# OpenHardware-Initiative/Drone-OA-IREE-ViT-Accelerator

Measured on AMD Instinct MI355X. Metric: frames/s on ITAViTLSTM int8, 60x90 depth input, higher is better.
Workload: dtype int8+f32; 1 GPU; ITAViTLSTM int8 end-to-end forward (BASELINE config 4): 1024 synthetic 60x90 depth frames per GPU per step, LSTM state carried, velocity all-gather; frames_per_gpu=1024, global_batch=1024, parallelism=dp1, image_dtype=u8, weights=seed-0 synthetic QAT (tests/golden), gather_every=1, gather=none (one GPU), schedule=one stream

## Files before the change

### drone-oa-iree-vit-accelerator_amd/csrc/ita_f16x3_kernels.h

```cpp
#pragma once
#include <type_traits>
#include "ita_device.h"

typedef _Float16 f16x8 __attribute__((ext_vector_type(8)));
typedef _Float16 f16x4 __attribute__((ext_vector_type(4)));
typedef float f32x16 __attribute__((ext_vector_type(16)));

__device__ __forceinline__ void split_f16(float x, _Float16& hi, _Float16& lo) {
  hi = (_Float16)x;
  lo = (_Float16)(x - (float)hi);
}

struct ItaGemmSplitArgs {
  const _Float16 *a_hi, *a_lo; int lda;
  const _Float16 *w_hi, *w_lo; int ldw;
  float* out;
  int M, N, K;
  int nsplit;
  int dbg;
  const _Float16 *wf_hi, *wf_lo;
};

template <int ROWS, int NT>
__device__ __forceinline__ void stage_plane(const _Float16* __restrict__ g, int ld, int row0, int max_row, int k0,
// ... 255 lines not shown
  }
  f32x4 xlast0 = {0.0f, 0.0f, 0.0f, 0.0f};
  float xlast1 = 0.0f;
  if (h == 0) {
    const f32x4 q = *(const f32x4*)(a.quat + (size_t)bc * 4);
    xlast0 = (f32x4){a.desvel[bc] / 10.0f, q.x, q.y, q.z};
    xlast1 = q.w;
  }
  const f32x4 ci = *(const f32x4*)(a.c_in + sb * 128 + u0);
  const f32x4 nh = *(const f32x4*)(a.nx_h_in + sb * 128 + u0);
  f32x4 bz[4];
#pragma unroll
  for (int gt = 0; gt < 4; ++gt) bz[gt] = *(const f32x4*)(a.bias + gt * 128 + u0);
  __builtin_amdgcn_sched_barrier(0);
#pragma unroll
  for (int i = 0; i < 4; ++i) {
    f32x4 ps = pz[0][i];
#pragma unroll
    for (int z = 1; z < NS; ++z) ps += pz[z][i];
    *(f32x4*)&pt[8 * i + (lane >> 3)][4 * (lane & 7)] = ps;
  }
#pragma unroll
  for (int i = 0; i < 16; ++i) *(f32x4*)&hs[2 * i + h][4 * r] = hv[i];
  __syncthreads();
#pragma unroll
  for (int s = 0; s < 9; ++s) {
    f32x4 x0 = xlast0, x1 = {xlast1, 0.0f, 0.0f, 0.0f};
    if (s < 8) {
      x0 = *(const f32x4*)&hs[r][16 * s + 8 * h];
      x1 = *(const f32x4*)&hs[r][16 * s + 8 * h + 4];
    }
    f16x8 xh, xl;
#pragma unroll
    for (int j = 0; j < 8; ++j) {
      const float x = j < 4 ? x0[j & 3] : x1[j & 3];
      const _Float16 hi = (_Float16)x;
      xh[j] = hi;
      xl[j] = (_Float16)(x - (float)hi);
    }
    acc = __builtin_amdgcn_mfma_f32_32x32x16_f16(wl[s], xh, acc, 0, 0, 0);
    acc = __builtin_amdgcn_mfma_f32_32x32x16_f16(wh[s], xl, acc, 0, 0, 0);
    acc = __builtin_amdgcn_mfma_f32_32x32x16_f16(wh[s], xh, acc, 0, 0, 0);
  }
  if (b >= a.B) return;
  f32x4 hn, cn;
#pragma unroll
  for (int q = 0; q < 4; ++q) {
    float g[4];
#pragma unroll
    for (int gt = 0; gt < 4; ++gt)
      g[gt] = (pt[r][gt * 8 + 4 * h + q] * a.inv_fold_scale + acc[4 * gt + q] * a.inv_wscale) + bz[gt][q];
    const float ig = lstm_sigmoid_fast(g[0]), fg = lstm_sigmoid_fast(g[1]), cg = lstm_tanh_fast(g[2]), og = lstm_sigmoid_fast(g[3]);
    const float c = fmaf(fg, ci[q], ig * cg);
    cn[q] = c;
    hn[q] = og * lstm_tanh_fast(c);
  }
  *(f32x4*)(a.c_out + sb * 128 + u0) = cn;
  *(f32x4*)(a.h_out + sb * 128 + u0) = hn;
  f16x4 h_hi, h_lo, n_hi, n_lo;
#pragma unroll
  for (int q = 0; q < 4; ++q) {
    _Float16 x, y;
    split_f16(hn[q], x, y); h_hi[q] = x; h_lo[q] = y;
    split_f16(nh[q], x, y); n_hi[q] = x; n_lo[q] = y;
  }
  const size_t o0 = ita_lstm_plane_index(b, u0), o1 = ita_lstm_plane_index(b, 128 + u0);
  *(f16x4*)(a.nx_hi + o0) = h_hi;
  *(f16x4*)(a.nx_lo + o0) = h_lo;
  *(f16x4*)(a.nx_hi + o1) = n_hi;
  *(f16x4*)(a.nx_lo + o1) = n_lo;
}

struct ItaLstmLayerArgs {
  const _Float16 *a_hi, *a_lo; int lda;
  const _Float16 *w_hi, *w_lo; int ldw;
  float inv_wscale;
  const float* bsum;
  const float* c_in;
  float *h_out, *c_out;
  _Float16 *nx_hi, *nx_lo;
  const float* nx_h_in;
  int B, K;
  const int* slots;
};
template <int NK>
__global__ __launch_bounds__(256) void ita_lstm_layer_kernel(const ItaLstmLayerArgs a) {
  __shared__ float part[4][16][64];
  const int tid = threadIdx.x, lane = tid & 63, wave = tid >> 6;
  const int ut = blockIdx.x, f0 = blockIdx.y * 32;
  static_assert(NK == 4, "fragment-order operands: four k-ranges of four k-steps (K = 256)");
  const size_t ao = ((size_t)((blockIdx.y * 4 + wave) * 4) * 64 + lane) * 8;
  const size_t wo = ((size_t)((ut * 4 + wave) * 4) * 64 + lane) * 8;
  f16x8 fah[NK], fal[NK], fwh[NK], fwl[NK];
#pragma unroll
  for (int s = 0; s < NK; ++s) {
    fwh[s] = *(const f16x8*)(a.w_hi + wo + 512 * s);
    fah[s] = *(const f16x8*)(a.a_hi + ao + 512 * s);
    fwl[s] = *(const f16x8*)(a.w_lo + wo + 512 * s);
    fal[s] = *(const f16x8*)(a.a_lo + ao + 512 * s);
  }
  const int ef = tid >> 3, eu = tid & 7;
  const int b = f0 + ef, u = ut * 8 + eu;
  const size_t sb = a.slots ? (size_t)a.slots[min(b, a.B - 1)] : (size_t)min(b, a.B - 1);
  const float c_prev = a.c_in[sb * 128 + u];
  const float nx_prev = a.nx_hi ? a.nx_h_in[sb * 128 + u] : 0.0f;
  const float b_i = a.bsum[u], b_f = a.bsum[128 + u], b_g = a.bsum[256 + u], b_o = a.bsum[384 + u];
  __builtin_amdgcn_sched_barrier(0);
  f32x16 acc;
#pragma unroll
  for (int e = 0; e < 16; ++e) acc[e] = 0.0f;
#pragma unroll
  for (int s = 0; s < NK; ++s) {
    acc = __builtin_amdgcn_mfma_f32_32x32x16_f16(fwl[s], fah[s], acc, 0, 0, 0);
    acc = __builtin_amdgcn_mfma_f32_32x32x16_f16(fwh[s], fal[s], acc, 0, 0, 0);
    acc = __builtin_amdgcn_mfma_f32_32x32x16_f16(fwh[s], fah[s], acc, 0, 0, 0);
  }
#pragma unroll
  for (int e = 0; e < 16; ++e) part[wave][e][lane] = acc[e];
  __syncthreads();
  if (b >= a.B) return;
  float gsum[4];
  const int pl = ef + 32 * (eu >> 2);
#pragma unroll
  for (int gte = 0; gte < 4; ++gte) {
    const int e = 4 * gte + (eu & 3);
    gsum[gte] = ((part[0][e][pl] + part[1][e][pl]) + part[2][e][pl]) + part[3][e][pl];
  }
  const float gi = gsum[0] * a.inv_wscale + b_i, gf = gsum[1] * a.inv_wscale + b_f,
              gg = gsum[2] * a.inv_wscale + b_g, go = gsum[3] * a.inv_wscale + b_o;
  const float ig = lstm_sigmoid_fast(gi), fg = lstm_sigmoid_fast(gf), cg = lstm_tanh_fast(gg), og = lstm_sigmoid_fast(go);
  const float c = fmaf(fg, c_prev, ig * cg);
  const float hn = og * lstm_tanh_fast(c);
  a.c_out[sb * 128 + u] = c;
  a.h_out[sb * 128 + u] = hn;
  if (a.nx_hi) {
    _Float16 x, y;
    const size_t o0 = ita_lstm_plane_index(b, u), o1 = ita_lstm_plane_index(b, 128 + u);
    split_f16(hn, x, y);
    a.nx_hi[o0] = x;
    a.nx_lo[o0] = y;
    split_f16(nx_prev, x, y);
    a.nx_hi[o1] = x;
    a.nx_lo[o1] = y;
  }
}

__global__ void ita_split_planes_kernel(const float* __restrict__ x, _Float16* __restrict__ hi, _Float16* __restrict__ lo,
                                        int width, int ld, int rows) {
  const size_t i8 = ((size_t)blockIdx.x * blockDim.x + threadIdx.x) * 8;
  if (i8 >= (size_t)rows * width) return;
  const size_t r = i8 / width, c = i8 - r * width;
  f16x8 vh, vl;
#pragma unroll
  for (int j = 0; j < 8; ++j) {
    _Float16 a, b;
    split_f16(x[i8 + j], a, b);
    vh[j] = a; vl[j] = b;
  }
  *(f16x8*)(hi + r * ld + c) = vh;
  *(f16x8*)(lo + r * ld + c) = vl;
}

__global__ void ita_impulse_kernel(float* x, int rows, int width, int col0) {
  const size_t idx = (size_t)blockIdx.x * blockDim.x + threadIdx.x;
  if (idx >= (size_t)rows * width) return;
  const int i = (int)(idx / width), c = (int)(idx % width);
  x[idx] = (c == col0 + i) ? 1.0f : 0.0f;
}

struct ItaTailBigArgs {
  const float* x;
  const _Float16 *w_hi, *w_lo;
  const float* bias;
  float inv_wscale;
  float* out;
  int B, E, TH, TW, CO, nchunk;
  int accumulate;
};
template <int NT, int WAVES, int TPS>
struct ItaTailBigLds {
  static constexpr int HP = (2 * WAVES + 2) * 34;
  static constexpr int A_PLANE = HP * 64;
  static constexpr int W_PLANE = TPS * NT * 16 * 64;
  static constexpr int AH = 0, AL = A_PLANE, WH = 2 * A_PLANE, WL = WH + W_PLANE;
  static constexpr int GEO_I = WL + W_PLANE;
  static constexpr int GEO_F = GEO_I + HP * 16;
  static constexpr int TOTAL = GEO_F + HP * 8;
};

template <int NT, int WAVES, int TPS>
__global__ __launch_bounds__(64 * WAVES) void ita_tail_big_kernel(const ItaTailBigArgs a) {
  using L = ItaTailBigLds<NT, WAVES, TPS>;
  static_assert(9 % TPS == 0, "taps per weight stage must divide 9");
  constexpr int W_CHUNK_HALVES = 9 * NT * 16 * 32;
  constexpr int NTHR = 64 * WAVES;
  extern __shared__ __attribute__((aligned(16))) char lds[];
  const int tid = threadIdx.x, lane = tid & 63, wave = tid >> 6;
  const int OH = 2 * a.TH, OW = 2 * a.TW, C4 = a.E / 4, CIN = C4 + a.E;
  const int tx0 = blockIdx.x * 32, ty0 = blockIdx.y * 2 * WAVES, b = blockIdx.z;
  const float* xt = a.x + (size_t)b * a.TH * a.TW * a.E;
  const float sy = (float)(a.TH - 1) / (float)(OH - 1), sx = (float)(a.TW - 1) / (float)(OW - 1);

  f32x4 acc[4][NT];
#pragma unroll
  for (int mt = 0; mt < 4; ++mt)
#pragma unroll
    for (int nt = 0; nt < NT; ++nt) acc[mt][nt] = (f32x4){0.0f, 0.0f, 0.0f, 0.0f};

  for (int p = tid; p < L::HP; p += NTHR) {
    const int hy = p / 34, hx = p - 34 * hy;
    const int y = ty0 + hy - 1, x = tx0 + hx - 1;
    const int ok = (y >= 0 && y < OH && x >= 0 && x < OW) ? 4 : 0;
    const int yc = min(max(y, 0), OH - 1), xc = min(max(x, 0), OW - 1);
    const float fy = sy * (float)yc, fx = sx * (float)xc;
    int y0 = (int)fy, x0 = (int)fx;
    if (y0 > a.TH - 1) y0 = a.TH - 1;
    if (x0 > a.TW - 1) x0 = a.TW - 1;
    const int yp = y0 < a.TH - 1 ? 2 : 0, xp = x0 < a.TW - 1 ? 1 : 0;
    *(i32x4*)(lds + L::GEO_I + p * 16) = (i32x4){(y0 * a.TW + x0) * a.E,
                                                   ((yc >> 1) * a.TW + (xc >> 1)) * a.E + 2 * (yc & 1) + (xc & 1), ok | yp | xp, 0};
    *(f32x2*)(lds + L::GEO_F + p * 8) = (f32x2){fy - (float)y0, fx - (float)x0};
  }

  for (int ch = 0; ch < a.nchunk; ++ch) {
    __syncthreads();
    auto stage_w = [&](int tap0) {
// ... 455 lines not shown
```

### drone-oa-iree-vit-accelerator_amd/csrc/ita_plugin.hip

```cpp
#include <hip/hip_runtime.h>

#include <cstdio>
#include <cstdlib>
#include <cstring>
#include <mutex>
#include <string>
#include <atomic>
#include <functional>
#include <thread>
#include <vector>

#include "../../include/ita_mi355x.h"
#include "../../include/ita_weights.h"
#include "../../include/ita_wire.h"
#include "ita_f16x3_kernels.h"
#include "ita_f32_kernels.h"
#include "ita_int8_kernels.h"
#include "ita_stream_kernel.h"
#include "ita_long_attn_kernel.h"
#include "ita_ffn_f32_kernel.h"
#include "ita_attn_f32_kernel.h"
#include "ita_ffn_f32_e128_kernel.h"
#include "ita_attn_f32_e128_kernel.h"

namespace {

thread_local int tl_err = ITA_OK;
thread_local std::string tl_msg;

int fail(int code, const std::string& msg) {
  tl_err = code;
  tl_msg = msg;
  return code;
}
#define HIPCHK(expr)                                                                              \
  do {                                                                                            \
    hipError_t e_ = (expr);                                                                       \
    if (e_ != hipSuccess)                                                                         \
      return fail(ITA_ERR_HIP, std::string(#expr) + ": " + hipGetErrorString(e_));                \
  } while (0)

constexpr int K0P = 672;
constexpr int K0S = 144;
constexpr int NSPLIT = 8;

struct Layer {
  const int8_t *wq, *wk, *wv, *wo, *w1, *w2;
  const int32_t *bq, *bk, *bv, *bo, *b1, *b2;
  float ascal[ITA_A_NSCAL], fscal[ITA_F_NSCAL];
  const float *n1w, *n1b, *n2w, *n2b;
  bool ffn_f32 = false;
  const float *w1f = nullptr, *b1f = nullptr, *w2f = nullptr, *b2f = nullptr;
  float *w1p = nullptr, *w2p = nullptr;
  bool attn_f32 = false;
  const float *wqf = nullptr, *wkf = nullptr, *wvf = nullptr, *bqf = nullptr, *bkf = nullptr, *bvf = nullptr,
              *wof = nullptr, *bof = nullptr;
  char *simg_enc = nullptr, *simg_tok = nullptr, *simg_mha = nullptr;
  unsigned fast_sites = 0;
};

}

struct ita_context {
  int device = 0;
  int num_cus = 256;
  bool loaded = false;
  ita_blob_header hdr{};
  std::vector<char> hblob;
  char* dblob = nullptr;
  std::vector<Layer> layers;
  const float *tail_b = nullptr, *dec_w = nullptr, *dec_b = nullptr, *fc_w = nullptr, *fc_b = nullptr;
  float* tail_wT = nullptr;
  char* tok_simg = nullptr;
  size_t tok_simg_bytes = 0;
  float* wcat[3] = {nullptr, nullptr, nullptr};
  float* bsum[3] = {nullptr, nullptr, nullptr};
  int kfold = 8192, ldfold = 8192 + 64;
  int tail_mode = 1;
  bool folded = false;
  _Float16 *foldf_hi = nullptr, *foldf_lo = nullptr;
  _Float16 *fold_hi = nullptr, *fold_lo = nullptr;
  float* fold_bias = nullptr;
  float fold_inv_scale = 1.0f;
  _Float16 *lw_hi[3] = {nullptr, nullptr, nullptr}, *lw_lo[3] = {nullptr, nullptr, nullptr};
  float lw_inv_scale[3] = {1.0f, 1.0f, 1.0f};
  _Float16 *x2_hi = nullptr, *x2_lo = nullptr, *c1_hi = nullptr, *c1_lo = nullptr,
           *c2_hi = nullptr, *c2_lo = nullptr;
  float* part = nullptr;
  int cap = 0;
  bool ws_reserved = false;
  int front_cap[ITA_PART_BUFFERS] = {};
  float *bufA = nullptr, *bufB = nullptr, *cat0 = nullptr, *cat1 = nullptr, *cat2 = nullptr, *gates = nullptr,
        *feat = nullptr;
  bool prof = false;
  int prof_max = 0, prof_n = 0;
  int prof_every = 1, prof_stage = -1, prof_calls = 0;
  std::vector<hipEvent_t> prof_ev;
  std::vector<hipEvent_t> pipe_ev;
  float* pipe_h = nullptr;
  int pipe_cap = 0;
  _Float16 *tl_hi = nullptr, *tl_lo = nullptr;
  _Float16 *tu_hi = nullptr, *tu_lo = nullptr;
  _Float16 *ts_hi = nullptr, *ts_lo = nullptr;
  float* tl_bias = nullptr;
  float tl_inv_scale = 1.0f;
  int tl_E = 0, tl_CO = 0, tl_nt = 0, tl_nchunk = 0;
  char* long_ws = nullptr;
  size_t long_ws_bytes = 0;
  float *dsp_in = nullptr, *dsp_out = nullptr;
  std::vector<float> dsp_host;
};

namespace {

std::mutex g_bind_mu;
ita_handle g_bound = nullptr;
int g_bound_layer = 0;
int g_bound_dtype = ITA_DISPATCH_F16;

template <typename T>
const T* dptr(ita_context* c, const char* name, bool required, bool* ok) {
  const ita_blob_entry* e = ita_blob_find(c->hblob.data(), c->hblob.size(), name);
  if (!e) {
    if (required) *ok = false;
    return nullptr;
  }
  return (const T*)(c->dblob + e->offset);
}
template <typename T>
const T* hptr(ita_context* c, const char* name) {
  const ita_blob_entry* e = ita_blob_find(c->hblob.data(), c->hblob.size(), name);
  return e ? (const T*)(c->hblob.data() + e->offset) : nullptr;
}

void free_weights(ita_context* c) {
  for (Layer& L : c->layers) {
    char** im[] = {&L.simg_enc, &L.simg_tok, &L.simg_mha};
    for (char** q : im) {
      if (*q) (void)hipFree(*q);
      *q = nullptr;
    }
    float** fim[] = {&L.w1p, &L.w2p};
    for (float** q : fim) {
      if (*q) (void)hipFree(*q);
      *q = nullptr;
    }
  }
  if (c->dblob) (void)hipFree(c->dblob);
  if (c->tail_wT) (void)hipFree(c->tail_wT);
  if (c->tok_simg) (void)hipFree(c->tok_simg);
  c->tok_simg = nullptr;
  for (int l = 0; l < 3; ++l) {
    if (c->wcat[l]) (void)hipFree(c->wcat[l]);
    if (c->bsum[l]) (void)hipFree(c->bsum[l]);
    c->wcat[l] = c->bsum[l] = nullptr;
  }
  void* extra[] = {c->foldf_hi, c->foldf_lo, c->fold_hi, c->fold_lo, c->fold_bias, c->lw_hi[0], c->lw_lo[0], c->lw_hi[1], c->lw_lo[1],
                   c->lw_hi[2], c->lw_lo[2]};
  for (void* q : extra)
    if (q) (void)hipFree(q);
  c->fold_hi = c->fold_lo = c->foldf_hi = c->foldf_lo = nullptr;
  c->fold_bias = nullptr;
  for (int l = 0; l < 3; ++l) c->lw_hi[l] = c->lw_lo[l] = nullptr;
  c->folded = false;
  c->dblob = nullptr;
  c->tail_wT = nullptr;
  c->loaded = false;
}

void free_workspace(ita_context* c) {
  float** bufs[] = {&c->bufA, &c->bufB, &c->cat0, &c->cat1, &c->cat2, &c->gates, &c->feat};
  for (float** b : bufs) {
    if (*b) (void)hipFree(*b);
    *b = nullptr;
  }
  _Float16** hb[] = {&c->x2_hi, &c->x2_lo, &c->c1_hi, &c->c1_lo, &c->c2_hi, &c->c2_lo};
  for (_Float16** b : hb) {
    if (*b) (void)hipFree(*b);
    *b = nullptr;
  }
  if (c->part) (void)hipFree(c->part);
  c->part = nullptr;
  c->cap = 0;
  for (int& fc : c->front_cap) fc = 0;
}

int ensure_workspace(ita_context* c, int B, hipStream_t s = nullptr) {
  if (B <= c->cap) return ITA_OK;
  if (c->ws_reserved)
    return fail(ITA_ERR_INVALID_ARG, "batch exceeds the workspace pinned by ita_reserve; call ita_reserve(max_batch) again while idle");
  hipStreamCaptureStatus cs = hipStreamCaptureStatusNone;
  if (hipStreamIsCapturing(s, &cs) == hipSuccess && cs != hipStreamCaptureStatusNone)
    return fail(ITA_ERR_INVALID_ARG, "the workspace cannot grow inside a stream capture; call ita_reserve first");
  free_workspace(c);
  const size_t E = (size_t)c->hdr.E;
  HIPCHK(hipMalloc(&c->bufA, sizeof(float) * B * 128 * E));
  HIPCHK(hipMalloc(&c->bufB, sizeof(float) * B * 128 * E));
  HIPCHK(hipMalloc(&c->feat, sizeof(float) * (size_t)B * 4608));
  HIPCHK(hipMalloc(&c->cat0, sizeof(float) * (size_t)B * K0P));
  HIPCHK(hipMalloc(&c->cat1, sizeof(float) * (size_t)B * 256));
  HIPCHK(hipMalloc(&c->cat2, sizeof(float) * (size_t)B * 256));
  HIPCHK(hipMalloc(&c->gates, sizeof(float) * (size_t)B * 512));
  HIPCHK(hipMalloc(&c->x2_hi, 2 * 2 * (size_t)B * c->ldfold));
  HIPCHK(hipMalloc(&c->x2_lo, 2 * 2 * (size_t)B * c->ldfold));
  HIPCHK(hipMalloc(&c->c1_hi, 2 * (size_t)((B + 31) / 32 * 32) * 256));
  HIPCHK(hipMalloc(&c->c1_lo, 2 * (size_t)((B + 31) / 32 * 32) * 256));
  HIPCHK(hipMalloc(&c->c2_hi, 2 * (size_t)((B + 31) / 32 * 32) * 256));
  HIPCHK(hipMalloc(&c->c2_lo, 2 * (size_t)((B + 31) / 32 * 32) * 256));
  HIPCHK(hipMalloc(&c->part, ITA_PART_BUFFERS * sizeof(float) * (size_t)NSPLIT * B * 512));
  c->cap = B;
  return ITA_OK;
}

template <typename K>
int set_lds(K kernel, int bytes) {
  HIPCHK(hipFuncSetAttribute(reinterpret_cast<const void*>(kernel), hipFuncAttributeMaxDynamicSharedMemorySize, bytes));
  return ITA_OK;
}

int check(ita_handle h, int batch, bool need_weights = true) {
  if (!h) return fail(ITA_ERR_INVALID_ARG, "null handle");
  if (batch <= 0) return fail(ITA_ERR_INVALID_ARG, "batch must be positive");
  if (need_weights && !h->loaded) return fail(ITA_ERR_NO_WEIGHTS, "ita_load_weights has not been called");
  HIPCHK(hipSetDevice(h->device));
  return ITA_OK;
}

ItaMhaArgs mha_args(ita_context* c, int layer, const float* x, float* y, int B, bool fuse, const ita_mha_taps* t) {
  const Layer& L = c->layers[layer];
  ItaMhaArgs a{};
  a.x = x; a.y = y;
  a.wq = L.wq; a.wk = L.wk; a.wv = L.wv; a.wo = L.wo;
  a.bq = L.bq; a.bk = L.bk; a.bv = L.bv; a.bo = L.bo;
  a.inv_sx = L.ascal[ITA_A_INV_SX]; a.mq = L.ascal[ITA_A_MQ]; a.mk = L.ascal[ITA_A_MK]; a.mv = L.ascal[ITA_A_MV];
  a.ml = L.ascal[ITA_A_ML]; a.mc = L.ascal[ITA_A_MC]; a.mo = L.ascal[ITA_A_MO]; a.so = L.ascal[ITA_A_SO];
  a.ln_w = L.n1w; a.ln_b = L.n1b;
  a.B = B; a.fuse_ln = fuse ? 1 : 0;
  if (t) {
    a.t_xq = t->x_q; a.t_Q = t->Q; a.t_K = t->K; a.t_V = t->V; a.t_logits = t->logits; a.t_probs = t->probs;
    a.t_ctx = t->ctx; a.t_out = t->out_q;
  }
  return a;
}

struct StreamIo;
int launch_stream(ita_context* c, int layer, int mode, bool fuse_ln, const StreamIo& io, int B, hipStream_t s);
int launch_mha_stream(ita_context* c, int layer, const float* x, float* y, int B, bool fuse, hipStream_t s);

int launch_mha(ita_context* c, int layer, const float* x, float* y, int B, bool fuse, const ita_mha_taps* t,
               hipStream_t s) {
  if (c->layers[layer].attn_f32)
    return fail(ITA_ERR_UNSUPPORTED, "this layer's attention is float32 (ITAW0003 blob): ita_mha_f32 runs it");
  if (fuse && !c->layers[layer].n1w) return fail(ITA_ERR_BAD_BLOB, "norm1 parameters missing from the blob");
  if (!t && c->layers[layer].simg_mha) return launch_mha_stream(c, layer, x, y, B, fuse, s);
  const ItaMhaArgs a = mha_args(c, layer, x, y, B, fuse, t);
  const int grid = B < c->num_cus ? B : c->num_cus;
  if (c->hdr.E == 64) {
    hipLaunchKernelGGL(ita_mha_kernel<64>, dim3(grid), dim3(512), ItaMhaLds<64>::TOTAL, s, a);
  } else {
    hipLaunchKernelGGL(ita_mha_kernel<128>, dim3(grid), dim3(512), ItaMhaLds<128>::TOTAL, s, a);
  }
  HIPCHK(hipGetLastError());
  return ITA_OK;
}

int launch_ffn(ita_context* c, int layer, const float* x, float* y, int B, bool fuse, const ita_ffn_taps* t,
               hipStream_t s, _Float16* y_hi = nullptr, _Float16* y_lo = nullptr) {
  const Layer& L = c->layers[layer];
  if (L.ffn_f32) return fail(ITA_ERR_UNSUPPORTED, "this layer's FFN is float32 (ITAW0002 blob): ita_ffn_f32 runs it");
  if (fuse && !L.n2w) return fail(ITA_ERR_BAD_BLOB, "norm2 parameters missing from the blob");
  ItaFfnArgs a{};
  a.x = x; a.y = y; a.w1 = L.w1; a.w2 = L.w2; a.b1 = L.b1; a.b2 = L.b2;
  a.inv_sx = L.fscal[ITA_F_INV_SX]; a.m1 = L.fscal[ITA_F_M1]; a.m2 = L.fscal[ITA_F_M2]; a.s2 = L.fscal[ITA_F_S2];
  a.ln_w = L.n2w; a.ln_b = L.n2b; a.B = B; a.fuse_ln = fuse ? 1 : 0;
  if (t) { a.t_xq = t->x_q; a.t_h = t->h; a.t_out = t->out_q; }
  a.y_hi = y_hi; a.y_lo = y_lo; a.ld_planes = c->ldfold;
  const int grid = B < 2 * c->num_cus ? B : 2 * c->num_cus;
  if (c->hdr.E == 64) {
    hipLaunchKernelGGL(ita_ffn_kernel<64>, dim3(grid), dim3(512), ItaFfnLds<64>::TOTAL, s, a);
  } else {
    hipLaunchKernelGGL(ita_ffn_kernel<128>, dim3(grid), dim3(512), ItaFfnLds<128>::TOTAL, s, a);
  }
  HIPCHK(hipGetLastError());
  return ITA_OK;
}

int launch_ffn_f32(ita_context* c, int layer, const float* x, float* y, int B, bool fuse, hipStream_t s,
                   _Float16* y_hi = nullptr, _Float16* y_lo = nullptr, const float* h0_src = nullptr, float* h0_dst = nullptr,
                   const int* slots = nullptr) {
  const Layer& L = c->layers[layer];
  if (!L.ffn_f32) return fail(ITA_ERR_UNSUPPORTED, "this layer's FFN is int8 (ITAW0001 blob): ita_ffn_int8 runs it");
  if (c->hdr.E != 64 && !L.w1p) return fail(ITA_ERR_UNSUPPORTED, "the float32 FFN of an ITAW0002 blob is built for E = 64");
// ... 1100 lines not shown
static int forward_impl(ita_handle h, const void* image, int image_dtype, const float* desvel, const float* quat,
                        const float* h_in, const float* c_in, float* vel, float* h_out, float* c_out, int batch,
                        const ita_forward_taps* taps, void* stream, const int* slots, int state_rows,
                        const float* x2_in = nullptr) {
  int rc = check(h, batch);
  if (rc) return rc;
  if ((!image && !x2_in) || !desvel || !quat || !h_in || !c_in || !vel || !h_out || !c_out)
    return fail(ITA_ERR_INVALID_ARG, "null pointer");
  if (image_dtype != ITA_IMAGE_F32 && image_dtype != ITA_IMAGE_U8) return fail(ITA_ERR_INVALID_ARG, "bad image dtype");
  if (!h->dec_w || !h->wcat[0] || !h->fc_w || (h->hdr.has_tail && !h->tail_wT))
    return fail(ITA_ERR_BAD_BLOB, "blob holds no decoder / LSTM (/ fusion tail) parameters");
  if (h->hdr.has_tail && h->hdr.E != 64) return fail(ITA_ERR_UNSUPPORTED, "the fusion tail is built for E = 64 (ITAViTLSTM)");
  if ((rc = ensure_workspace(h, batch, (hipStream_t)stream))) return rc;
  hipStream_t s = (hipStream_t)stream;
  const int B = batch;
  const size_t tokb = sizeof(float) * (size_t)B * 128 * h->hdr.E;
  const bool fast = h->tail_mode == 1 && h->folded;
  if (slots && !fast) return fail(ITA_ERR_UNSUPPORTED, "slot-indexed state needs tail mode 1");
  const size_t lstride = (size_t)(slots ? state_rows : batch) * 128;
  const bool stage_h0 = slots || (h_out < h_in + lstride && h_in < h_out + lstride);
  const int ev_per_fwd = 5 + 2 * h->hdr.num_layers;
  hipEvent_t* ev = nullptr;
  if (h->prof && h->prof_n < h->prof_max && (h->prof_calls++ % h->prof_every) == 0)
    ev = &h->prof_ev[(size_t)h->prof_n * ev_per_fwd];
  int evi = 0, m_lo = 0, m_hi = ev_per_fwd - 1;
  if (h->prof_stage >= 0) {
    const int L2 = 2 * h->hdr.num_layers;
    const int lo[ITA_NUM_STAGES] = {0, 1, 1, 1 + L2, 2 + L2, 3 + L2}, hi[ITA_NUM_STAGES] = {1, 1 + L2, 1 + L2, 2 + L2, 3 + L2, 4 + L2};
    m_lo = lo[h->prof_stage]; m_hi = hi[h->prof_stage];
  }
#define MARK() do { if (ev && (h->prof_stage < 0 || evi == m_lo || evi == m_hi)) HIPCHK(hipEventRecord(ev[evi], s)); ++evi; } while (0)
  MARK();
  const bool fused_tok = !x2_in && fuse_tokenizer(h, image_dtype);
  if (slots && !x2_in) {
    const Layer& LL = h->layers.back();
    if (!LL.ffn_f32 && !((fused_tok && h->hdr.num_layers == 1) ? LL.simg_tok : LL.simg_enc))
      return fail(ITA_ERR_UNSUPPORTED, "slot-indexed state needs the stream kernel (this blob's accumulator range rules it out)");
  }
  if (x2_in) {
    HIPCHK(hipMemcpyAsync(h->bufA, x2_in, tokb, hipMemcpyDeviceToDevice, s));
    if (fast) {
      const size_t n = (size_t)B * 128 * h->hdr.E;
      hipLaunchKernelGGL(ita_split_planes_kernel, dim3((unsigned)((n / 8 + 255) / 256)), dim3(256), 0, s, h->bufA, h->x2_hi,
                         h->x2_lo, 128 * h->hdr.E, h->ldfold, B);
      HIPCHK(hipGetLastError());
    }
    if (stage_h0) HIPCHK(hipMemcpyAsync(h->gates, h_in, sizeof(float) * (size_t)B * 128, hipMemcpyDeviceToDevice, s));
  } else if (!fused_tok && (rc = launch_tokenizer(h, image, image_dtype, h->bufA, B, s))) return rc;
  MARK();
  if (!x2_in && !fused_tok && taps && taps->tokens) HIPCHK(hipMemcpyAsync(taps->tokens, h->bufA, tokb, hipMemcpyDeviceToDevice, s));
  for (int l = 0; l < (x2_in ? 0 : h->hdr.num_layers); ++l) {
    const bool last = l == h->hdr.num_layers - 1;
    const bool planes = fast && last;
    float* yout = (planes && !(taps && taps->x2)) ? nullptr : h->bufA;
    bool marked = false;
    const std::function<int()> mid = [&]() -> int { MARK(); marked = true; return ITA_OK; };
    if ((rc = launch_encoder(h, l, h->bufA, yout, planes ? h->x2_hi : nullptr, planes ? h->x2_lo : nullptr,
                             (taps && last) ? taps->x1 : nullptr, B, s, nullptr, (planes && stage_h0) ? h_in : nullptr,
                             (planes && stage_h0) ? h->gates : nullptr, slots, (fused_tok && l == 0) ? image : nullptr,
                             (fused_tok && l == 0 && taps) ? taps->tokens : nullptr, &mid))) return rc;
    if (!marked) MARK();
    MARK();
  }
  if (x2_in) { MARK(); MARK(); }
  if (taps && taps->x2) HIPCHK(hipMemcpyAsync(taps->x2, h->bufA, tokb, hipMemcpyDeviceToDevice, s));
  if (fast) {
    if ((rc = launch_gemm_split<128, 128, 2, 4>(h->x2_hi, h->x2_lo, h->ldfold, h->fold_hi, h->fold_lo, h->ldfold, h->part, B,
                                                512, h->kfold, NSPLIT, s, h->foldf_hi, h->foldf_lo))) return rc;
    MARK();
    MARK();
    _Float16* chi[3] = {nullptr, h->c1_hi, h->c2_hi};
    _Float16* clo[3] = {nullptr, h->c1_lo, h->c2_lo};
    {
      ItaLstm0Args p{h->part, NSPLIT, h->fold_inv_scale, h->lw_hi[0], h->lw_lo[0], h->lw_inv_scale[0], h->fold_bias,
                     desvel, quat, stage_h0 ? h->gates  : h_in, c_in, h_out, c_out, chi[1], clo[1],
                     h_in + lstride, B, slots};
      hipLaunchKernelGGL(ita_lstm0_kernel<NSPLIT>, dim3(16, (B + 31) / 32), dim3(64), 0, s, p);
      HIPCHK(hipGetLastError());
    }
    for (int l = 1; l < 3; ++l) {
      ItaLstmLayerArgs p{chi[l], clo[l], 256, h->lw_hi[l], h->lw_lo[l], 256, h->lw_inv_scale[l], h->bsum[l],
                         c_in + l * lstride, h_out + l * lstride, c_out + l * lstride,
                         l < 2 ? chi[l + 1] : nullptr, l < 2 ? clo[l + 1] : nullptr,
                         l < 2 ? h_in + (l + 1) * lstride : nullptr, B, 256, slots};
      hipLaunchKernelGGL(ita_lstm_layer_kernel<4>, dim3(16, (B + 31) / 32), dim3(256), 0, s, p);
      HIPCHK(hipGetLastError());
    }
    hipLaunchKernelGGL(ita_fc_kernel, dim3((B * 3 + 63) / 64), dim3(64), 0, s, h_out + 2 * lstride, h->fc_w,
                       h->fc_b, vel, B, slots);
    HIPCHK(hipGetLastError());
    MARK();
  } else {
    if (h->hdr.has_tail) {
      if ((rc = launch_tail(h, h->bufA, h->feat, 4608, B, s))) return rc;
      MARK();
      if (taps && taps->feat)
        HIPCHK(hipMemcpyAsync(taps->feat, h->feat, sizeof(float) * (size_t)B * 4608, hipMemcpyDeviceToDevice, s));
      if ((rc = launch_gemm(h->feat, 4608, h->dec_w, 4608, h->dec_b, h->cat0, K0P, B, 512, 4608, s))) return rc;
    } else {
      MARK();
      if ((rc = launch_gemm(h->bufA, h->kfold, h->dec_w, h->kfold, h->dec_b, h->cat0, K0P, B, 512, h->kfold, s))) return rc;
    }
    MARK();
    if (taps && taps->dec)
      HIPCHK(hipMemcpy2DAsync(taps->dec, 512 * sizeof(float), h->cat0, K0P * sizeof(float), 512 * sizeof(float), B,
                              hipMemcpyDeviceToDevice, s));
    {
      ItaLstmPrepArgs p{desvel, quat, h_in, h->cat0, h->cat1, h->cat2, K0P, B};
      hipLaunchKernelGGL(ita_lstm_prep_kernel, dim3(B), dim3(256), 0, s, p);
      HIPCHK(hipGetLastError());
    }
    float* cats[3] = {h->cat0, h->cat1, h->cat2};
    const int kp[3] = {K0P, 256, 256};
    for (int l = 0; l < 3; ++l) {
      if ((rc = launch_gemm(cats[l], kp[l], h->wcat[l], kp[l], h->bsum[l], h->gates, 512, B, 512, kp[l], s))) return rc;
      ItaLstmPointArgs p{h->gates, c_in + (size_t)l * B * 128, h_out + (size_t)l * B * 128, c_out + (size_t)l * B * 128,
                         l < 2 ? cats[l + 1] : nullptr, 256, B};
      hipLaunchKernelGGL(ita_lstm_point_kernel, dim3((B * 128 + 255) / 256), dim3(256), 0, s, p);
      HIPCHK(hipGetLastError());
    }
    hipLaunchKernelGGL(ita_fc_kernel, dim3((B * 3 + 63) / 64), dim3(64), 0, s, h_out + (size_t)2 * B * 128, h->fc_w,
                       h->fc_b, vel, B);
    HIPCHK(hipGetLastError());
    MARK();
  }
#undef MARK
  if (ev) ++h->prof_n;
  return ITA_OK;
}

int ita_vitlstm_forward(ita_handle h, const void* image, int image_dtype, const float* desvel, const float* quat,
                        const float* h_in, const float* c_in, float* vel, float* h_out, float* c_out, int batch,
                        const ita_forward_taps* taps, void* stream) {
  return forward_impl(h, image, image_dtype, desvel, quat, h_in, c_in, vel, h_out, c_out, batch, taps, stream, nullptr, 0);
}

int ita_vitlstm_tail(ita_handle h, const float* x2, const float* desvel, const float* quat, const float* h_in,
                     const float* c_in, float* vel, float* h_out, float* c_out, int batch, void* stream) {
  if (!x2) return fail(ITA_ERR_INVALID_ARG, "null pointer");
  return forward_impl(h, nullptr, ITA_IMAGE_F32, desvel, quat, h_in, c_in, vel, h_out, c_out, batch, nullptr, stream, nullptr, 0, x2);
}

static int front_impl(ita_handle h, const void* image, int image_dtype, int batch, int buf, void* stream,
                      void* encoder_done_event, int xbuf = 0, int parts = 3) {
  int rc = check(h, batch);
  if (rc) return rc;
  if (((parts & 1) && !image) || buf < 0 || buf >= ITA_PART_BUFFERS || xbuf < 0 || xbuf > 1)
    return fail(ITA_ERR_INVALID_ARG, "null image, buf not in [0, ITA_PART_BUFFERS) or plane set not 0 / 1");
  if ((parts & 1) && image_dtype != ITA_IMAGE_F32 && image_dtype != ITA_IMAGE_U8) return fail(ITA_ERR_INVALID_ARG, "bad image dtype");
  if (!(h->tail_mode == 1 && h->folded)) return fail(ITA_ERR_UNSUPPORTED, "front/back form needs tail mode 1 and a full ITAViTLSTM blob");
  if ((rc = ensure_workspace(h, batch, (hipStream_t)stream))) return rc;
  if (parts & 2) h->front_cap[buf] = h->cap;
  hipStream_t s = (hipStream_t)stream;
  _Float16* const xh = h->x2_hi + (size_t)xbuf * h->cap * h->ldfold;
  _Float16* const xl = h->x2_lo + (size_t)xbuf * h->cap * h->ldfold;
  const int L2 = 2 * h->hdr.num_layers, per = 5 + L2;
  hipEvent_t* ev = nullptr;
  if (h->prof && h->prof_stage >= 0 && h->prof_n < h->prof_max && (h->prof_calls++ % h->prof_every) == 0)
    ev = &h->prof_ev[(size_t)h->prof_n * per];
  auto mark = [&](int stage, bool end) -> int {
    if (ev && h->prof_stage == stage) {
      const int lo[ITA_NUM_STAGES] = {0, 1, 1, 1 + L2, 2 + L2, 3 + L2}, hi[ITA_NUM_STAGES] = {1, 1 + L2, 1 + L2, 2 + L2, 3 + L2, 4 + L2};
      HIPCHK(hipEventRecord(ev[end ? hi[stage] : lo[stage]], s));
    }
    return ITA_OK;
  };
  if (parts & 1) {
    if ((rc = mark(0, false))) return rc;
    const bool fused_tok = fuse_tokenizer(h, image_dtype);
    if (!fused_tok && (rc = launch_tokenizer(h, image, image_dtype, h->bufA, batch, s))) return rc;
    if ((rc = mark(0, true)) || (rc = mark(1, false))) return rc;
    for (int l = 0; l < h->hdr.num_layers; ++l) {
      const bool last = l == h->hdr.num_layers - 1;
      if ((rc = launch_encoder(h, l, h->bufA, last ? nullptr : h->bufA, last ? xh : nullptr, last ? xl : nullptr,
                               nullptr, batch, s, nullptr, nullptr, nullptr, nullptr, (fused_tok && l == 0) ? image : nullptr,
                               nullptr))) return rc;
    }
    if ((rc = mark(1, true))) return rc;
    if (encoder_done_event) HIPCHK(hipEventRecord((hipEvent_t)encoder_done_event, s));
  }
  if (parts & 2) {
    if ((rc = mark(3, false))) return rc;
    float* part = h->part + (size_t)buf * NSPLIT * h->cap * 512;
    if ((rc = launch_gemm_split<128, 128, 2, 4>(xh, xl, h->ldfold, h->fold_hi, h->fold_lo, h->ldfold, part, batch, 512,
                                                h->kfold, NSPLIT, s, h->foldf_hi, h->foldf_lo))) return rc;
    if ((rc = mark(3, true))) return rc;
  }
  if (ev && (h->prof_stage == 0 || h->prof_stage == 1 || h->prof_stage == 3)) ++h->prof_n;
  return ITA_OK;
}

int ita_vitlstm_front(ita_handle h, const void* image, int image_dtype, int batch, int buf, void* stream) {
  return front_impl(h, image, image_dtype, batch, buf, stream, nullptr);
}

int ita_vitlstm_front_ev(ita_handle h, const void* image, int image_dtype, int batch, int buf, void* stream,
                         void* encoder_done_event) {
  return front_impl(h, image, image_dtype, batch, buf, stream, encoder_done_event);
}

int ita_vitlstm_encode(ita_handle h, const void* image, int image_dtype, int batch, int plane_set, void* stream) {
  return front_impl(h, image, image_dtype, batch, 0, stream, nullptr, plane_set, 1);
}

int ita_vitlstm_fold(ita_handle h, int batch, int plane_set, int buf, void* stream) {
  return front_impl(h, nullptr, ITA_IMAGE_U8, batch, buf, stream, nullptr, plane_set, 2);
}

int ita_vitlstm_back(ita_handle h, const float* desvel, const float* quat, const float* h_in, const float* c_in, float* vel,
                     float* h_out, float* c_out, int batch, int buf, void* stream) {
  int rc = check(h, batch);
  if (rc) return rc;
  if (!desvel || !quat || !h_in || !c_in || !vel || !h_out || !c_out || buf < 0 || buf >= ITA_PART_BUFFERS)
    return fail(ITA_ERR_INVALID_ARG, "null pointer or buf not in [0, ITA_PART_BUFFERS)");
  if (!(h->tail_mode == 1 && h->folded)) return fail(ITA_ERR_UNSUPPORTED, "front/back form needs tail mode 1 and a full ITAViTLSTM blob");
  if (batch > h->cap || h->front_cap[buf] != h->cap)
    return fail(ITA_ERR_INVALID_ARG, "ita_vitlstm_front has not filled this buffer for the current workspace (reserve before front)");
  hipStream_t s = (hipStream_t)stream;
  const int B = batch;
  const size_t lstride = (size_t)B * 128;
  const float* part = h->part + (size_t)buf * NSPLIT * h->cap * 512;
  const bool stage_h0 = h_out < h_in + lstride && h_in < h_out + lstride;
  if (stage_h0) HIPCHK(hipMemcpyAsync(h->gates, h_in, sizeof(float) * lstride, hipMemcpyDeviceToDevice, s));
  {
    ItaLstm0Args p{part, NSPLIT, h->fold_inv_scale, h->lw_hi[0], h->lw_lo[0], h->lw_inv_scale[0], h->fold_bias, desvel, quat,
                   stage_h0 ? h->gates : h_in, c_in, h_out, c_out, h->c1_hi, h->c1_lo, h_in + lstride, B, nullptr};
    hipLaunchKernelGGL(ita_lstm0_kernel<NSPLIT>, dim3(16, (B + 31) / 32), dim3(64), 0, s, p);
    HIPCHK(hipGetLastError());
  }
  _Float16* chi[3] = {nullptr, h->c1_hi, h->c2_hi};
  _Float16* clo[3] = {nullptr, h->c1_lo, h->c2_lo};
  for (int l = 1; l < 3; ++l) {
    ItaLstmLayerArgs p{chi[l], clo[l], 256, h->lw_hi[l], h->lw_lo[l], 256, h->lw_inv_scale[l], h->bsum[l],
                       c_in + l * lstride, h_out + l * lstride, c_out + l * lstride, l < 2 ? chi[l + 1] : nullptr,
                       l < 2 ? clo[l + 1] : nullptr, l < 2 ? h_in + (l + 1) * lstride : nullptr, B, 256, nullptr};
    hipLaunchKernelGGL(ita_lstm_layer_kernel<4>, dim3(16, (B + 31) / 32), dim3(256), 0, s, p);
    HIPCHK(hipGetLastError());
  }
  hipLaunchKernelGGL(ita_fc_kernel, dim3((B * 3 + 63) / 64), dim3(64), 0, s, h_out + 2 * lstride, h->fc_w, h->fc_b, vel, B,
                     (const int*)nullptr);
  HIPCHK(hipGetLastError());
  return ITA_OK;
}

int ita_vitlstm_pipelined(ita_handle h, const void* const* image, int image_dtype, const float* const* desvel,
                          const float* const* quat, float* state_h, float* state_c, float* const* vel, int batch, int n_steps,
                          void* stream_front, void* stream_back) {
  int rc = check(h, batch);
  if (rc) return rc;
  if (!image || !desvel || !quat || !state_h || !state_c || !vel || n_steps <= 0 || !stream_front || !stream_back ||
      stream_front == stream_back)
    return fail(ITA_ERR_INVALID_ARG, "null argument, n_steps <= 0, or the two streams are not two distinct non-default streams");
  if (h->prof)
    return fail(ITA_ERR_INVALID_ARG, "ita_vitlstm_pipelined cannot run between ita_profile_begin and ita_profile_end");
  if ((rc = ensure_workspace(h, batch, (hipStream_t)stream_front))) return rc;
  hipStream_t sf = (hipStream_t)stream_front, sb = (hipStream_t)stream_back;
  const size_t nstate = (size_t)3 * batch * 128;
  if (h->pipe_cap < batch) {
    if (h->pipe_h) (void)hipFree(h->pipe_h);
    h->pipe_h = nullptr; h->pipe_cap = 0;
    HIPCHK(hipMalloc(&h->pipe_h, 2 * nstate * sizeof(float)));
    h->pipe_cap = batch;
  }
  while ((int)h->pipe_ev.size() < 2 * ITA_PART_BUFFERS + 1) {
    hipEvent_t e;
    HIPCHK(hipEventCreateWithFlags(&e, hipEventDisableTiming));
    h->pipe_ev.push_back(e);
  }
  hipEvent_t* evf = h->pipe_ev.data();
  hipEvent_t* evb = h->pipe_ev.data() + ITA_PART_BUFFERS;
  float* sh[2] = {state_h, h->pipe_h};
  float* sc[2] = {state_c, h->pipe_h + nstate};
  HIPCHK(hipEventRecord(h->pipe_ev[2 * ITA_PART_BUFFERS], sf));
  HIPCHK(hipStreamWaitEvent(sb, h->pipe_ev[2 * ITA_PART_BUFFERS], 0));
  std::atomic<int> fronts_recorded{0}, backs_recorded{0}, abort_flag{0};
  int rc_back = ITA_OK;
  std::string msg_back;
  auto back_body = [&]() {
    if (hipSetDevice(h->device) != hipSuccess) {
      rc_back = fail(ITA_ERR_HIP, "hipSetDevice (back stream's host thread)");
      msg_back = tl_msg;
      abort_flag.store(1, std::memory_order_relaxed);
      return;
    }
    for (int t = 0; t < n_steps; ++t) {
      const int buf = t % ITA_PART_BUFFERS;
      while (fronts_recorded.load(std::memory_order_acquire) <= t) {
        if (abort_flag.load(std::memory_order_relaxed)) return;
        std::this_thread::yield();
      }
      if (hipStreamWaitEvent(sb, evf[buf], 0) != hipSuccess) { rc_back = fail(ITA_ERR_HIP, "hipStreamWaitEvent (back stream)"); break; }
      if ((rc_back = ita_vitlstm_back(h, desvel[t], quat[t], sh[t & 1], sc[t & 1], vel[t], sh[(t + 1) & 1], sc[(t + 1) & 1], batch,
                                      buf, sb)))
        break;
      if (hipEventRecord(evb[buf], sb) != hipSuccess) { rc_back = fail(ITA_ERR_HIP, "hipEventRecord (back stream)"); break; }
      backs_recorded.store(t + 1, std::memory_order_release);
    }
    if (rc_back) {
      msg_back = tl_msg;
      abort_flag.store(1, std::memory_order_relaxed);
    }
  };
  std::thread back_thread;
  try {
    back_thread = std::thread(back_body);
  } catch (const std::exception& e) {
    return fail(ITA_ERR_HIP, std::string("ita_vitlstm_pipelined: cannot start the back stream's host thread: ") + e.what());
  }
  for (int t = 0; t < n_steps && !rc; ++t) {
    const int buf = t % ITA_PART_BUFFERS;
    if (t >= ITA_PART_BUFFERS) {
      while (backs_recorded.load(std::memory_order_acquire) <= t - ITA_PART_BUFFERS && !abort_flag.load(std::memory_order_relaxed))
        std::this_thread::yield();
      if (abort_flag.load(std::memory_order_relaxed)) break;
      if (hipStreamWaitEvent(sf, evb[buf], 0) != hipSuccess) { rc = fail(ITA_ERR_HIP, "hipStreamWaitEvent (front stream)"); break; }
    }
    if ((rc = ita_vitlstm_front(h, image[t], image_dtype, batch, buf, sf))) break;
    if (hipEventRecord(evf[buf], sf) != hipSuccess) { rc = fail(ITA_ERR_HIP, "hipEventRecord (front stream)"); break; }
    fronts_recorded.store(t + 1, std::memory_order_release);
  }
  if (rc) abort_flag.store(1, std::memory_order_relaxed);
  back_thread.join();
  if (rc) return rc;
  if (rc_back) return fail(rc_back, "ita_vitlstm_pipelined, back stream's host thread: " + msg_back);
// ... 195 lines not shown
```

Measured before the change: 10.69 million frames/s.

## Fuse final FC head into last LSTM layer via last-block-done counter

The last LSTM layer kernel now writes each hidden value into a per-batch-tile slab and bumps an atomic counter per tile. The last block to finish a tile loads the full 128-unit hidden tile and weights into shared memory and computes the 3-output velocity FC directly. This removes the separate FC kernel launch and its reread of h_out. In exchange it adds atomics, fences, a slab buffer and a counter that must reset correctly, and the FC runs serially in a single block per tile.

Result: no change. 10.78 million frames/s (median of 6 runs) (+0.8%).

```diff
diff --git a/drone-oa-iree-vit-accelerator_amd/csrc/ita_f16x3_kernels.h b/drone-oa-iree-vit-accelerator_amd/csrc/ita_f16x3_kernels.h
--- a/drone-oa-iree-vit-accelerator_amd/csrc/ita_f16x3_kernels.h
+++ b/drone-oa-iree-vit-accelerator_amd/csrc/ita_f16x3_kernels.h
@@ -361,8 +361,13 @@
   const float* nx_h_in;
   int B, K;
   const int* slots;
+  const float *fc_w, *fc_b;
+  float* vel;
+  float* fc_slab;
+  int* fc_cnt;
 };
-template <int NK>
+constexpr int ITA_FC_CNT_STRIDE = 64;
+template <int NK, bool FC = false>
 __global__ __launch_bounds__(256) void ita_lstm_layer_kernel(const ItaLstmLayerArgs a) {
   __shared__ float part[4][16][64];
   const int tid = threadIdx.x, lane = tid & 63, wave = tid >> 6;
@@ -397,30 +402,72 @@
 #pragma unroll
   for (int e = 0; e < 16; ++e) part[wave][e][lane] = acc[e];
   __syncthreads();
-  if (b >= a.B) return;
-  float gsum[4];
-  const int pl = ef + 32 * (eu >> 2);
-#pragma unroll
-  for (int gte = 0; gte < 4; ++gte) {
-    const int e = 4 * gte + (eu & 3);
-    gsum[gte] = ((part[0][e][pl] + part[1][e][pl]) + part[2][e][pl]) + part[3][e][pl];
-  }
-  const float gi = gsum[0] * a.inv_wscale + b_i, gf = gsum[1] * a.inv_wscale + b_f,
-              gg = gsum[2] * a.inv_wscale + b_g, go = gsum[3] * a.inv_wscale + b_o;
-  const float ig = lstm_sigmoid_fast(gi), fg = lstm_sigmoid_fast(gf), cg = lstm_tanh_fast(gg), og = lstm_sigmoid_fast(go);
-  const float c = fmaf(fg, c_prev, ig * cg);
-  const float hn = og * lstm_tanh_fast(c);
-  a.c_out[sb * 128 + u] = c;
-  a.h_out[sb * 128 + u] = hn;
-  if (a.nx_hi) {
-    _Float16 x, y;
-    const size_t o0 = ita_lstm_plane_index(b, u), o1 = ita_lstm_plane_index(b, 128 + u);
-    split_f16(hn, x, y);
-    a.nx_hi[o0] = x;
-    a.nx_lo[o0] = y;
-    split_f16(nx_prev, x, y);
-    a.nx_hi[o1] = x;
-    a.nx_lo[o1] = y;
+  if (b < a.B) {
+    float gsum[4];
+    const int pl = ef + 32 * (eu >> 2);
+#pragma unroll
+    for (int gte = 0; gte < 4; ++gte) {
+      const int e = 4 * gte + (eu & 3);
+      gsum[gte] = ((part[0][e][pl] + part[1][e][pl]) + part[2][e][pl]) + part[3][e][pl];
+    }
+    const float gi = gsum[0] * a.inv_wscale + b_i, gf = gsum[1] * a.inv_wscale + b_f,
+                gg = gsum[2] * a.inv_wscale + b_g, go = gsum[3] * a.inv_wscale + b_o;
+    const float ig = lstm_sigmoid_fast(gi), fg = lstm_sigmoid_fast(gf), cg = lstm_tanh_fast(gg), og = lstm_sigmoid_fast(go);
+    const float c = fmaf(fg, c_prev, ig * cg);
+    const float hn = og * lstm_tanh_fast(c);
+    a.c_out[sb * 128 + u] = c;
+    a.h_out[sb * 128 + u] = hn;
+    if (a.nx_hi) {
+      _Float16 x, y;
+      const size_t o0 = ita_lstm_plane_index(b, u), o1 = ita_lstm_plane_index(b, 128 + u);
+      split_f16(hn, x, y);
+      a.nx_hi[o0] = x;
+      a.nx_lo[o0] = y;
+      split_f16(nx_prev, x, y);
+      a.nx_hi[o1] = x;
+      a.nx_lo[o1] = y;
+    }
+    if constexpr (FC)
+      __hip_atomic_store(a.fc_slab + (size_t)blockIdx.y * 4096 + u * 32 + ef, hn, __ATOMIC_RELAXED, __HIP_MEMORY_SCOPE_AGENT);
+  }
+  if constexpr (FC) {
+    __shared__ int last;
+    __shared__ float wfc[3 * 128 + 3];
+    asm volatile("s_waitcnt vmcnt(0)" ::: "memory");
+    __syncthreads();
+    if (tid == 0) {
+      int* const cnt = a.fc_cnt + (size_t)blockIdx.y * ITA_FC_CNT_STRIDE;
+      const bool l = __hip_atomic_fetch_add(cnt, 1, __ATOMIC_RELAXED, __HIP_MEMORY_SCOPE_AGENT) == (int)gridDim.x - 1;
+      if (l) {
+        __builtin_amdgcn_fence(__ATOMIC_ACQUIRE, "agent");
+        asm volatile("s_waitcnt vmcnt(0)" ::: "memory");
+        __hip_atomic_store(cnt, 0, __ATOMIC_RELAXED, __HIP_MEMORY_SCOPE_AGENT);
+      }
+      last = l;
+    }
+    __syncthreads();
+    if (!last) return;
+    const __amdgpu_buffer_rsrc_t slab =
+        __builtin_amdgcn_make_buffer_rsrc(a.fc_slab + (size_t)blockIdx.y * 4096, 0, 4096 * sizeof(float), 0x00020000);
+    f32x4 hv[4];
+#pragma unroll
+    for (int i = 0; i < 4; ++i)
+      hv[i] = __builtin_bit_cast(f32x4, __builtin_amdgcn_raw_buffer_load_b128(slab, (i * 256 + tid) * 16, 0, 16));
+    const float w0 = a.fc_w[tid], w1 = tid < 128 ? a.fc_w[256 + tid] : 0.0f, bv = tid < 3 ? a.fc_b[tid] : 0.0f;
+    wfc[tid] = w0;
+    if (tid < 128) wfc[256 + tid] = w1;
+    if (tid < 3) wfc[3 * 128 + tid] = bv;
+    float* const hs = &part[0][0][0];
+#pragma unroll
+    for (int i = 0; i < 4; ++i) *(f32x4*)(hs + (i * 256 + tid) * 4) = hv[i];
+    __syncthreads();
+    if (tid < 96) {
+      const int o = tid >> 5, fb = f0 + (tid & 31);
+      float acc = wfc[3 * 128 + o];
+#pragma unroll 16
+      for (int k = 0; k < 128; ++k) acc = fmaf(hs[k * 32 + (tid & 31)], wfc[o * 128 + k], acc);
+      if (fb < a.B) a.vel[(size_t)fb * 3 + o] = acc;
+    }
   }
 }
 
diff --git a/drone-oa-iree-vit-accelerator_amd/csrc/ita_plugin.hip b/drone-oa-iree-vit-accelerator_amd/csrc/ita_plugin.hip
--- a/drone-oa-iree-vit-accelerator_amd/csrc/ita_plugin.hip
+++ b/drone-oa-iree-vit-accelerator_amd/csrc/ita_plugin.hip
@@ -87,6 +87,8 @@
   _Float16 *x2_hi = nullptr, *x2_lo = nullptr, *c1_hi = nullptr, *c1_lo = nullptr,
            *c2_hi = nullptr, *c2_lo = nullptr;
   float* part = nullptr;
+  float* fc_slab = nullptr;
+  int* fc_cnt = nullptr;
   int cap = 0;
   bool ws_reserved = false;
   int front_cap[ITA_PART_BUFFERS] = {};
@@ -181,6 +183,10 @@
   }
   if (c->part) (void)hipFree(c->part);
   c->part = nullptr;
+  if (c->fc_slab) (void)hipFree(c->fc_slab);
+  if (c->fc_cnt) (void)hipFree(c->fc_cnt);
+  c->fc_slab = nullptr;
+  c->fc_cnt = nullptr;
   c->cap = 0;
   for (int& fc : c->front_cap) fc = 0;
 }
@@ -208,6 +214,11 @@
   HIPCHK(hipMalloc(&c->c2_hi, 2 * (size_t)((B + 31) / 32 * 32) * 256));
   HIPCHK(hipMalloc(&c->c2_lo, 2 * (size_t)((B + 31) / 32 * 32) * 256));
   HIPCHK(hipMalloc(&c->part, ITA_PART_BUFFERS * sizeof(float) * (size_t)NSPLIT * B * 512));
+  const size_t ntile = (size_t)(B + 31) / 32;
+  HIPCHK(hipMalloc(&c->fc_slab, sizeof(float) * ntile * 4096));
+  HIPCHK(hipMalloc(&c->fc_cnt, sizeof(int) * ntile * ITA_FC_CNT_STRIDE));
+  HIPCHK(hipMemsetAsync(c->fc_cnt, 0, sizeof(int) * ntile * ITA_FC_CNT_STRIDE, s));
+  HIPCHK(hipStreamSynchronize(s));
   c->cap = B;
   return ITA_OK;
 }
@@ -1474,13 +1485,12 @@
       ItaLstmLayerArgs p{chi[l], clo[l], 256, h->lw_hi[l], h->lw_lo[l], 256, h->lw_inv_scale[l], h->bsum[l],
                          c_in + l * lstride, h_out + l * lstride, c_out + l * lstride,
                          l < 2 ? chi[l + 1] : nullptr, l < 2 ? clo[l + 1] : nullptr,
-                         l < 2 ? h_in + (l + 1) * lstride : nullptr, B, 256, slots};
-      hipLaunchKernelGGL(ita_lstm_layer_kernel<4>, dim3(16, (B + 31) / 32), dim3(256), 0, s, p);
+                         l < 2 ? h_in + (l + 1) * lstride : nullptr, B, 256, slots,
+                         h->fc_w, h->fc_b, vel, h->fc_slab, h->fc_cnt};
+      if (l < 2) hipLaunchKernelGGL(ita_lstm_layer_kernel<4>, dim3(16, (B + 31) / 32), dim3(256), 0, s, p);
+      else hipLaunchKernelGGL((ita_lstm_layer_kernel<4, true>), dim3(16, (B + 31) / 32), dim3(256), 0, s, p);
       HIPCHK(hipGetLastError());
     }
-    hipLaunchKernelGGL(ita_fc_kernel, dim3((B * 3 + 63) / 64), dim3(64), 0, s, h_out + 2 * lstride, h->fc_w,
-                       h->fc_b, vel, B, slots);
-    HIPCHK(hipGetLastError());
     MARK();
   } else {
     if (h->hdr.has_tail) {
@@ -1625,13 +1635,12 @@
   for (int l = 1; l < 3; ++l) {
     ItaLstmLayerArgs p{chi[l], clo[l], 256, h->lw_hi[l], h->lw_lo[l], 256, h->lw_inv_scale[l], h->bsum[l],
                        c_in + l * lstride, h_out + l * lstride, c_out + l * lstride, l < 2 ? chi[l + 1] : nullptr,
-                       l < 2 ? clo[l + 1] : nullptr, l < 2 ? h_in + (l + 1) * lstride : nullptr, B, 256, nullptr};
-    hipLaunchKernelGGL(ita_lstm_layer_kernel<4>, dim3(16, (B + 31) / 32), dim3(256), 0, s, p);
+                       l < 2 ? clo[l + 1] : nullptr, l < 2 ? h_in + (l + 1) * lstride : nullptr, B, 256, nullptr,
+                       h->fc_w, h->fc_b, vel, h->fc_slab, h->fc_cnt};
+    if (l < 2) hipLaunchKernelGGL(ita_lstm_layer_kernel<4>, dim3(16, (B + 31) / 32), dim3(256), 0, s, p);
+    else hipLaunchKernelGGL((ita_lstm_layer_kernel<4, true>), dim3(16, (B + 31) / 32), dim3(256), 0, s, p);
     HIPCHK(hipGetLastError());
   }
-  hipLaunchKernelGGL(ita_fc_kernel, dim3((B * 3 + 63) / 64), dim3(64), 0, s, h_out + 2 * lstride, h->fc_w, h->fc_b, vel, B,
-                     (const int*)nullptr);
-  HIPCHK(hipGetLastError());
   return ITA_OK;
 }
 
```
